# joedownard/skill-chaining-with-graphs

Measured on AMD Instinct MI355X. Metric: env-steps/sec (whole node), 65 536 parallel Pinball envs at 1/2/4/8 MI355X, higher is better.
Workload: dtype f32

## Files before the change

skill-chaining-with-graphs_amd/csrc/scg_kernels.hip:

```cpp
#include "scg_device.hpp"
#include "../../include/scg_abi.h"
#include <cstdio>
#include <cstdlib>
#include <cstring>
#include <cmath>
#include <mutex>
#include <new>
#include <type_traits>
#include <vector>

using namespace scg;
typedef float f4v __attribute__((ext_vector_type(4)));
typedef unsigned u4v __attribute__((ext_vector_type(4)));

#include "scg_eval.hpp"
#include "scg_step_kernel.hpp"
#include "scg_rollout_kernel.hpp"
#include "scg_trial_kernel.hpp"
#include "scg_order.hpp"
#include "scg_collect_kernels.hpp"
#include "scg_reduce_kernel.hpp"
#include "scg_apply_kernels.hpp"
#include "scg_aux_kernels.hpp"

// ... 142 lines not shown
    if (!c || !c->h_async) return 0;
    const uint32_t w = *reinterpret_cast<volatile uint32_t *>(c->h_async);
    if (w == 0) return 0;
    decode_async(w, c->err, sizeof(c->err));
    return 1;
}

extern "C" {

int scg_abi_version(void) { return SCG_ABI_VERSION; }

int scg_decode_async_word(uint32_t word, char *buf, int32_t buf_len) {
    return decode_async(word, buf, buf_len > 0 ? (size_t)buf_len : 0);
}

int scg_async_status(scg_ctx *c, void *stream, int32_t synchronize, uint32_t *word_out) {
    if (!c) return fail(nullptr, SCG_ERR_INVALID, "scg_async_status: null ctx");
    if (synchronize) {
        SCG_ON_DEVICE(c, "scg_async_status");
        SCG_HIP(c, hipStreamSynchronize(reinterpret_cast<hipStream_t>(stream)));
    }
    const uint32_t w = c->h_async ? *reinterpret_cast<volatile uint32_t *>(c->h_async) : 0u;
    if (word_out) *word_out = w;
    return decode_async(w, c->err, sizeof(c->err));
}

int scg_clear_async_error(scg_ctx *c) {
    if (!c) return fail(nullptr, SCG_ERR_INVALID, "scg_clear_async_error: null ctx");
    if (c->h_async) *reinterpret_cast<volatile uint32_t *>(c->h_async) = 0u;
    if (c->d_fail) {
        DeviceGuard g(c->cfg.device);
        if (g.ok) (void)hipMemset(c->d_fail, 0, sizeof(int32_t));
    }
    c->order_valid = false; c->hist_dirty = true; c->arm_rows_ready = false;
    return SCG_OK;
}

static int set_timeout(scg_ctx *c, const char *fn, double scg_ctx::*field, double seconds) {
    if (!c) return fail_in(nullptr, SCG_ERR_INVALID, fn, "null ctx");
    if (!(seconds >= 0.0) || seconds > 3600.0) return fail_in(c, SCG_ERR_INVALID, fn, "seconds must be in [0, 3600]");
    c->*field = seconds;
    return SCG_OK;
}

int scg_set_fit_timeout(scg_ctx *c, double seconds) { return set_timeout(c, "scg_set_fit_timeout", &scg_ctx::fit_timeout_s, seconds); }

int scg_set_peer_timeout(scg_ctx *c, double seconds) { return set_timeout(c, "scg_set_peer_timeout", &scg_ctx::peer_timeout_s, seconds); }

int scg_debug_raise_async(scg_ctx *c, uint32_t word) {
    if (!c || !c->h_async) return fail(c, SCG_ERR_INVALID, "scg_debug_raise_async: null ctx");
    *reinterpret_cast<volatile uint32_t *>(c->h_async) |= word;
    return SCG_OK;
}

int scg_block_envs(void) { return BLOCK_ENVS; }

const char *scg_strerror(int status) {
    switch (status) {
        case SCG_OK: return "ok";
        case SCG_ERR_INVALID: return "invalid argument";
        case SCG_ERR_NO_DEVICE: return "no usable HIP device";
        case SCG_ERR_HIP: return "HIP runtime error";
        case SCG_ERR_STATE: return "call order / state error";
        case SCG_ERR_ASYNC: return "an earlier launch failed on the device";
        default: return "unknown status";
    }
}

const char *scg_last_error(const scg_ctx *ctx) { return ctx ? ctx->err : g_err; }

static size_t hist_bytes(const scg_ctx *c) { return (size_t)((c->cfg.n_envs + 255) / 256) * HSTRIDE * sizeof(int32_t); }

struct CtxAlloc { void **ptr; size_t bytes; bool zero; };
static std::vector<CtxAlloc> ctx_allocs(scg_ctx *c) {
    auto P = [](auto **p) { return reinterpret_cast<void **>(p); };
    const size_t w = (size_t)c->n_vf * NACT * NF * sizeof(float), npos = (size_t)c->nblk * BLOCK_ENVS;
    const size_t rows = (size_t)(c->cfg.n_envs + COL_ROW - 1) / COL_ROW + 1;
    return {
        {P(&c->d_slabs), (size_t)c->nblk * w, false},
        {P(&c->d_cnts), (size_t)c->nblk * c->n_vf * sizeof(int32_t), true},
        {P(&c->d_G), w, true},
        {P(&c->d_nk), MAX_VF * sizeof(int32_t), true},
        {P(&c->d_edges), MAX_EDGES * 8 * sizeof(float), false},
        {P(&c->d_scale), NF * sizeof(float), false},
        {P(&c->d_perm), npos * sizeof(int32_t), false},
        {P(&c->d_hist), hist_bytes(c), false},
        {P(&c->d_collect_rows), rows * sizeof(int32_t), false},
        {P(&c->d_frontier_rows), MAX_VF * rows * sizeof(int32_t), false},
        {P(&c->d_fit_part), (size_t)FIT_BATCH * 2 * FIT_G * 8 * sizeof(unsigned long long), false},
        {P(&c->d_fail), sizeof(int32_t), true},
        {P(&c->d_outrec), npos * OREC * sizeof(float4), false},
        {P(&c->d_qalt), npos * 2 * sizeof(float4), false},
        {P(&c->d_invperm), npos * sizeof(int32_t), false},
        {P(&c->d_hist2[0]), hist_bytes(c), true},
        {P(&c->d_hist2[1]), hist_bytes(c), true},
        {P(&c->d_cellmask), (size_t)CELL_G * CELL_G * 4 * sizeof(uint64_t), false},
    };
}

#ifdef SCG_REDUCE_STAMPS
static size_t reduce_stamp_bytes(const scg_ctx *c) {
    const int nrow = (c->cfg.n_envs + 255) / 256, sy = (nrow + RED_NCOL - 1) / RED_NCOL;
    return (size_t)RED_NCOL * (c->n_vf + sy) * RED_STAMP_SLOTS * sizeof(unsigned long long);
}
#endif

int scg_create(scg_ctx **out, const scg_config *cfg) {
    if (!out || !cfg) return fail(nullptr, SCG_ERR_INVALID, "scg_create: null argument");
    *out = nullptr;
    if (cfg->n_envs < 1) return fail(nullptr, SCG_ERR_INVALID, "scg_create: n_envs must be >= 1");
    if (cfg->n_options < 0 || cfg->n_options > SCG_MAX_OPTIONS)
        return fail(nullptr, SCG_ERR_INVALID, "scg_create: n_options out of range [0,5]");
    if (cfg->update_count_floor < 0) return fail(nullptr, SCG_ERR_INVALID, "scg_create: update_count_floor must be >= 0");
    if (cfg->reoffer_period != 0 && !pow2(cfg->reoffer_period))
        return fail(nullptr, SCG_ERR_INVALID, "scg_create: reoffer_period must be a power of two (or 0)");
    if (cfg->fourier_order != SCG_FOURIER_ORDER)
        return fail(nullptr, SCG_ERR_INVALID, "scg_create: only Fourier order 5 is built");
    int ndev = 0;
    if (hipGetDeviceCount(&ndev) != hipSuccess || ndev < 1)
        return fail(nullptr, SCG_ERR_NO_DEVICE, "scg_create: no HIP device visible");
    if (cfg->device < 0 || cfg->device >= ndev)
        return fail(nullptr, SCG_ERR_INVALID, "scg_create: device ordinal out of range");
    scg_ctx *c = new (std::nothrow) scg_ctx();
    if (!c) return fail(nullptr, SCG_ERR_INVALID, "scg_create: out of host memory");
    memset(c, 0, sizeof(*c));
    c->cfg = *cfg;
    c->n_vf = cfg->n_options + 1;
    c->nblk = (cfg->n_envs + BLOCK_ENVS - 1) / BLOCK_ENVS;
    if (hipDeviceGetAttribute(&c->n_cu, hipDeviceAttributeMultiprocessorCount, cfg->device) != hipSuccess || c->n_cu <= 0) c->n_cu = 256;
    int st = SCG_OK;
    DeviceGuard dev_guard_(cfg->device);
    do {
        if (!dev_guard_.ok) { st = SCG_ERR_HIP; break; }
        for (const CtxAlloc &a : ctx_allocs(c)) {
            if (hipMalloc(a.ptr, a.bytes) != hipSuccess || (a.zero && hipMemset(*a.ptr, 0, a.bytes) != hipSuccess)) { st = SCG_ERR_HIP; break; }
        }
        if (st != SCG_OK) break;
        if (hipHostMalloc(reinterpret_cast<void **>(&c->h_async), 64, hipHostMallocMapped) != hipSuccess) { st = SCG_ERR_HIP; break; }
        *c->h_async = 0u;
        if (hipHostGetDevicePointer(reinterpret_cast<void **>(&c->d_async), c->h_async, 0) != hipSuccess) { st = SCG_ERR_HIP; break; }
    } while (0);
    if (st != SCG_OK) {
        snprintf(g_err, 256, "scg_create: device allocation/setup failed: %s", hipGetErrorString(hipGetLastError()));
        scg_destroy(c);
        return st;
    }
#ifdef SCG_STAMPS_LITE
    if (hipMalloc(&c->d_stamps, (size_t)c->nblk * STAMP_SLOTS * sizeof(unsigned long long)) == hipSuccess)
        (void)hipMemset(c->d_stamps, 0, (size_t)c->nblk * STAMP_SLOTS * sizeof(unsigned long long));
#endif
#ifdef SCG_REDUCE_STAMPS
    if (hipMalloc(&c->d_stamps, reduce_stamp_bytes(c)) == hipSuccess) (void)hipMemset(c->d_stamps, 0, reduce_stamp_bytes(c));
#endif
    c->parents = 0;
    for (int k = 1; k < MAX_VF; ++k) c->parents |= (uint32_t)(k - 1) << (3 * k);
    c->G_out = c->d_G; c->nk_out = c->d_nk;
    c->fit_timeout_s = 2.0;
    c->peer_timeout_s = 2.0;
    *out = c;
    return SCG_OK;
}

int scg_destroy(scg_ctx *c) {
    if (!c) return SCG_OK;
    for (const CtxAlloc &a : ctx_allocs(c)) (void)hipFree(*a.ptr);
    (void)hipFree(c->d_starts);
    if (c->h_async) (void)hipHostFree(c->h_async);
    if (c->peer_region) {
        DeviceGuard g(c->cfg.device);
        for (int r = 0; r < PEER_MAX; ++r)
            if (c->peer_mapped[r]) (void)hipIpcCloseMemHandle(c->peer_base[r]);
        {
            std::lock_guard<std::mutex> lk(g_peer_mu);
            for (size_t i = 0; i < g_peer_regions.size(); ++i)
                if (g_peer_regions[i].second == c->peer_region) { g_peer_regions.erase(g_peer_regions.begin() + i); break; }
        }
        (void)hipFree(c->peer_region); (void)hipFree(c->d_peer_go);
    }
    if (c->prof_ev) {
        for (hipEvent_t e : *c->prof_ev) (void)hipEventDestroy(e);
        delete c->prof_ev;
    }
    delete c;
    return SCG_OK;
}

int scg_set_hparams(scg_ctx *c, float gamma, float alpha, float epsilon, float r_option_success,
                    int32_t max_episode_steps, int32_t max_option_steps, int32_t update_count_floor, int32_t reoffer_period) {
    if (!c) return fail(nullptr, SCG_ERR_INVALID, "scg_set_hparams: null ctx");
    if (update_count_floor < 0) return fail(c, SCG_ERR_INVALID, "scg_set_hparams: update_count_floor must be >= 0");
    if (reoffer_period != 0 && !pow2(reoffer_period)) return fail(c, SCG_ERR_INVALID, "scg_set_hparams: reoffer_period must be a power of two (or 0)");
    c->cfg.gamma = gamma; c->cfg.alpha = alpha; c->cfg.epsilon = epsilon;
    c->cfg.r_option_success = r_option_success;
    c->cfg.max_episode_steps = max_episode_steps; c->cfg.max_option_steps = max_option_steps;
    c->cfg.update_count_floor = update_count_floor;
    c->cfg.reoffer_period = reoffer_period;
    return SCG_OK;
}

int scg_set_map(scg_ctx *c, const float *edges, int32_t n_edges, const float *starts, int32_t n_starts,
                const float map_scalars[6], const float *scale) {
    if (!c) return fail(nullptr, SCG_ERR_INVALID, "scg_set_map: null ctx");
    if (!edges || !starts || !map_scalars || !scale) return fail(c, SCG_ERR_INVALID, "scg_set_map: null argument");
    if (n_edges < 0 || n_edges > MAX_EDGES) return fail(c, SCG_ERR_INVALID, "scg_set_map: n_edges out of range [0,256]");
    if (n_starts < 1) return fail(c, SCG_ERR_INVALID, "scg_set_map: need at least one start position");
    SCG_ON_DEVICE(c, "scg_set_map");
    if (c->d_starts) { (void)hipFree(c->d_starts); c->d_starts = nullptr; }
    SCG_HIP(c, hipMalloc(&c->d_starts, (size_t)n_starts * 2 * sizeof(float)));
    if (n_edges > 0) SCG_HIP(c, hipMemcpy(c->d_edges, edges, (size_t)n_edges * 8 * sizeof(float), hipMemcpyHostToDevice));
    SCG_HIP(c, hipMemcpy(c->d_starts, starts, (size_t)n_starts * 2 * sizeof(float), hipMemcpyHostToDevice));
    SCG_HIP(c, hipMemcpy(c->d_scale, scale, NF * sizeof(float), hipMemcpyHostToDevice));
    const float R = map_scalars[0];
    c->ms.hstep = map_scalars[1]; c->ms.R2 = map_scalars[2];
    c->ms.TX = map_scalars[3]; c->ms.TY = map_scalars[4]; c->ms.TR2 = map_scalars[5];
    c->ms.R = R; c->ms.TR = (float)(std::sqrt((double)map_scalars[5]) * 1.0001);
    {
        std::vector<uint64_t> cm((size_t)CELL_G * CELL_G * 4, 0);
        const double vmax = 2.0 * std::sqrt(2.0) * 1.001;
        const double reach = (double)R * (1.02 + 1.10 * vmax) * 1.01 + 0.5 * std::sqrt(2.0) / CELL_G + 1e-6;
        for (int cy = 0; cy < CELL_G; ++cy)
            for (int cx = 0; cx < CELL_G; ++cx) {
                const double px = (cx + 0.5) / CELL_G, py = (cy + 0.5) / CELL_G;
                for (int j = 0; j < n_edges; ++j) {
                    const float *E = edges + 8 * j;
                    const double dx = px - E[0], dy = py - E[1];
                    double t = (dx * E[2] + dy * E[3]) * E[4];
                    t = t < 0 ? 0 : (t > 1 ? 1 : t);
                    const double qx = E[0] + E[2] * t - px, qy = E[1] + E[3] * t - py;
                    if (std::sqrt(qx * qx + qy * qy) <= reach)
                        cm[((size_t)cy * CELL_G + cx) * 4 + (j >> 6)] |= (1ull << (j & 63));
                }
            }
        SCG_HIP(c, hipMemcpy(c->d_cellmask, cm.data(), cm.size() * sizeof(uint64_t), hipMemcpyHostToDevice));
    }
    c->ms.n_edges = n_edges; c->ms.n_starts = n_starts;
    c->have_map = true;
    return SCG_OK;
}

struct PeerTarget {
    scg_ctx *c;
    float *G, *nkf;
    int32_t *nk;
    explicit PeerTarget(scg_ctx *ctx) : c(ctx), G(ctx->G_out), nkf(ctx->nkf_out), nk(ctx->nk_out) {
        if (!c->peer_n) return;
        float *op = reinterpret_cast<float *>(c->peer_region + PEER_HDR + (c->peer_e & 1u) * c->peer_op_stride);
        c->G_out = op; c->nkf_out = op + (size_t)c->n_vf * NACT * NF; c->nk_out = c->d_nk;
    }
    ~PeerTarget() { c->G_out = G; c->nkf_out = nkf; c->nk_out = nk; }
};

extern "C++" template <typename Args>
static void fill_shared(const scg_ctx *c, Args &A) {
    memset(&A, 0, sizeof(A));
    A.n = c->cfg.n_envs; A.n_vf = c->n_vf;
    A.seed = c->cfg.seed; A.env_base = c->cfg.env_id_base;
    A.epsilon = c->cfg.epsilon; A.max_ep = c->cfg.max_episode_steps; A.max_opt = c->cfg.max_option_steps;
    A.reoffer_mask = c->cfg.reoffer_period > 1 ? (uint32_t)(c->cfg.reoffer_period - 1) : 0u;
    A.parents = c->parents; A.gest = c->gest;
    A.ms = c->ms;
    A.edges = c->d_edges; A.starts = c->d_starts; A.cellmask = c->d_cellmask;
}

static void fill_common(const scg_ctx *c, StepArgs &A) {
    fill_shared(c, A);
    A.gamma = c->cfg.gamma; A.r_succ = c->cfg.r_option_success;
    A.slabs = c->d_slabs; A.cnts = c->d_cnts;
    A.gest_succ = c->gest_succ;
    A.ring_x = c->ring_x; A.ring_y = c->ring_y; A.events = c->events; A.ev_len = c->ev_len;
    A.ring_mask = c->ring_len > 0 ? c->ring_len - 1 : 0;
    A.stamps = c->d_stamps;
    A.async_word = c->d_async; A.fail_flag = c->d_fail;
}

enum ReduceMode { REDUCE_ONLY, COMMIT_ONLY, REDUCE_COMMIT, REDUCE_COMMIT_SORT };
static int launch_reduce(scg_ctx *c, float *W, uint32_t apply, int nblk, hipStream_t s, ReduceMode mode, const StepArgs *st = nullptr) {
    ReduceArgs R;
    memset(&R, 0, sizeof(R));
    R.slabs = c->d_slabs; R.cnts = c->d_cnts; R.G = c->G_out; R.n_k = c->nk_out; R.nk_f = c->nkf_out; R.W = W; R.scale = c->d_scale;
    R.nblk = nblk; R.n_vf = c->n_vf; R.alpha = c->cfg.alpha; R.apply = apply; R.fail_flag = c->d_fail; R.nk_floor = c->cfg.update_count_floor;
    const int nrow = st ? (c->cfg.n_envs + 255) / 256 : 0;
    R.n = c->cfg.n_envs; R.nrow = nrow;
    if (st) {
        R.outrec = c->d_outrec; R.qalt = c->d_qalt; R.invperm = c->d_invperm; R.perm = c->d_perm; R.sort = mode == REDUCE_COMMIT_SORT ? 1 : 0;
        R.hist = c->d_hist2[c->hist_parity]; R.hist_zero = c->d_hist2[c->hist_parity ^ 1];
        R.x = st->x; R.y = st->y; R.vx = st->vx; R.vy = st->vy; R.reward = st->reward;
        R.option_id_out = st->option_id; R.opt_steps = st->opt_steps; R.ep_steps = st->ep_steps;
        R.action = st->action; R.done = st->done;
        R.qcache = st->k_hi >= 0 ? st->qcache : nullptr;
        if (c->arm_bits && c->events && c->ring_x) {
            R.c_events = c->events; R.c_prev = c->arm_prev; R.c_evlen = c->ev_len; R.c_count = c->arm_count;
            R.c_rows = c->d_collect_rows; R.c_bits = c->arm_bits; R.c_L = c->arm_L; R.c_ring_len = c->ring_len;
        }
    }
#ifdef SCG_REDUCE_STAMPS
    R.stamps = c->d_stamps;
#endif
    if (mode == COMMIT_ONLY) {
        hipLaunchKernelGGL(commit_kernel, dim3(nrow), dim3(256), 0, s, R);
        SCG_HIP(c, hipGetLastError());
        return SCG_OK;
    }
    const int sy = (nrow + RED_NCOL - 1) / RED_NCOL;
    if (RED_NCOL * (c->n_vf + sy) <= c->n_cu)
        hipLaunchKernelGGL(reduce_kernel<16>, dim3(RED_NCOL, c->n_vf + sy), dim3(RED_THREADS), 0, s, R);
    else
        hipLaunchKernelGGL(reduce_kernel<8>, dim3(RED_NCOL, c->n_vf + sy), dim3(RED_THREADS), 0, s, R);
    SCG_HIP(c, hipGetLastError());
    return SCG_OK;
}

static int sort_env_order(scg_ctx *c, const int32_t *option_id, hipStream_t s) {
    if (c->order_valid && c->order_ids == option_id) return SCG_OK;
    const int nrow = (c->cfg.n_envs + 255) / 256;
    hipLaunchKernelGGL(sort_hist_kernel, dim3(nrow), dim3(256), 0, s, option_id, c->cfg.n_envs, c->n_vf, c->d_hist);
    hipLaunchKernelGGL(sort_scatter_kernel, dim3(nrow), dim3(256), 0, s, option_id, c->cfg.n_envs, c->n_vf, nrow,
                       c->d_hist, c->d_perm, c->d_invperm);
    SCG_HIP(c, hipGetLastError());
    return SCG_OK;
}

static int prof_begin(scg_ctx *c, hipStream_t s, hipEvent_t &ev1) {
    if (!(c->prof_on && (c->prof_seen++ % c->prof_every) == c->prof_every / 2)) return SCG_OK;
    if (!c->prof_ev) c->prof_ev = new std::vector<hipEvent_t>();
    while (c->prof_ev->size() < c->prof_used + 2) {
        hipEvent_t e;
        SCG_HIP(c, hipEventCreate(&e));
        c->prof_ev->push_back(e);
    }
    hipEvent_t ev0 = (*c->prof_ev)[c->prof_used];
    ev1 = (*c->prof_ev)[c->prof_used + 1];
    c->prof_used += 2;
    SCG_HIP(c, hipEventRecord(ev0, s));
    return SCG_OK;
}

int scg_step(scg_ctx *c, float *x, float *y, float *vx, float *vy, int32_t *option_id, int32_t *opt_steps,
             int32_t *ep_steps, float *qcache, uint8_t *action, float *reward, uint8_t *done, float *W,
             const float *clf, uint32_t enabled_mask, uint64_t t, uint32_t flags, void *stream) {
    if (!c) return fail(nullptr, SCG_ERR_INVALID, "scg_step: null ctx");
    if (!c->have_map) return fail(c, SCG_ERR_STATE, "scg_step: scg_set_map has not been called");
    if (!x || !y || !vx || !vy || !option_id || !opt_steps || !ep_steps || !qcache || !action || !reward ||
        !done || !W || !clf)
        return fail(c, SCG_ERR_INVALID, "scg_step: null array argument");
    if (c->peer_n && (flags & SCG_STEP_LEARN) && (flags & SCG_STEP_APPLY))
        return fail(c, SCG_ERR_INVALID, "scg_step: SCG_STEP_APPLY with a peer region open (the update is scg_peer_exchange_apply's)");
    if ((flags & SCG_STEP_INTERRUPT) && !(flags & SCG_STEP_LEARN))
        return fail(c, SCG_ERR_INVALID, "scg_step: SCG_STEP_INTERRUPT without SCG_STEP_LEARN (acting-only interruption is scg_rollout_interrupt)");
    SCG_CHECK_ASYNC(c);
    SCG_ON_DEVICE(c, "scg_step");
    if (c->arm_bits) {
        const void *ptrs[2] = {c->arm_count, c->arm_prev};
        for (const void *p : ptrs) {
            if (!p) continue;
            hipPointerAttribute_t at;
            if (hipPointerGetAttributes(&at, p) != hipSuccess || at.type != hipMemoryTypeDevice) {
                (void)hipGetLastError();
                c->arm_bits = 0; c->arm_rows_ready = false;
                return fail(c, SCG_ERR_STATE, "scg_step: the buffers announced with scg_arm_collect are no longer device memory "
                                              "(freed before scg_arm_collect(0)?); the trigger has been disarmed");
            }
        }
    }
    hipStream_t s = reinterpret_cast<hipStream_t>(stream);
    StepArgs A;
    fill_common(c, A);
    A.x = x; A.y = y; A.vx = vx; A.vy = vy;
    A.option_id = option_id; A.opt_steps = opt_steps; A.ep_steps = ep_steps; A.qcache = qcache;
    A.action = action; A.reward = reward; A.done = done;
    A.W = W; A.clf = clf;
    A.k_lo = 0; A.k_hi = c->n_vf - 1;
    A.enabled = enabled_mask; A.learn = (flags & SCG_STEP_LEARN) ? 1u : 0u; A.t = t;
    if (flags & 0x100u) A.k_hi = -1;
    if (const int rc = sort_env_order(c, option_id, s)) return rc;
    c->order_valid = false;
    if (c->hist_dirty) {
        const size_t hb = hist_bytes(c);
        SCG_HIP(c, hipMemsetAsync(c->d_hist2[0], 0, hb, s));
        SCG_HIP(c, hipMemsetAsync(c->d_hist2[1], 0, hb, s));
        c->hist_dirty = false;
    }
    const bool fold = (flags & SCG_STEP_LEARN) && !(flags & 0x200u);
    A.hist_next = fold ? c->d_hist2[c->hist_parity] : nullptr;
    A.perm = c->d_perm; A.outrec = c->d_outrec; A.qalt = c->d_qalt;
    hipEvent_t ev1 = nullptr;
    if (const int rc = prof_begin(c, s, ev1)) return rc;
    if (flags & SCG_STEP_INTERRUPT)
        hipLaunchKernelGGL(td_kernel<MODE_FUSED_INT>, dim3(c->nblk), dim3(THREADS), 0, s, A);
    else
        hipLaunchKernelGGL(td_kernel<MODE_FUSED>, dim3(c->nblk), dim3(THREADS), 0, s, A);
    SCG_HIP(c, hipGetLastError());
    if (ev1) SCG_HIP(c, hipEventRecord(ev1, s));
    c->arm_rows_ready = c->arm_bits && c->events && c->ring_x;
    if (!(flags & SCG_STEP_LEARN)) return launch_reduce(c, W, 0u, c->nblk, s, COMMIT_ONLY, &A);
    PeerTarget peer_target(c);
    if (!fold) return launch_reduce(c, W, (flags & SCG_STEP_APPLY) ? 1u : 0u, c->nblk, s, REDUCE_COMMIT, &A);
    c->hist_dirty = true;
    const int rc = launch_reduce(c, W, (flags & SCG_STEP_APPLY) ? 1u : 0u, c->nblk, s, REDUCE_COMMIT_SORT, &A);
    if (rc != SCG_OK) return rc;
    c->hist_dirty = false;
    c->hist_parity ^= 1;
    c->order_valid = true; c->order_ids = option_id;
    return SCG_OK;
}

static bool rollout_epw(const scg_ctx *c, int n, int &epw) {
    epw = 2;
    while (epw < RO_MAX_EPW && (long long)n >= (long long)c->n_cu * RO_WAVES * epw * 2) epw *= 2;
    if (const char *ov = getenv("SCG_ROLLOUT_EPW")) {
        const int v = atoi(ov);
        if (v < 2 || v > RO_MAX_EPW || !pow2(v)) return false;
        epw = v;
    }
    return true;
}

static int check_record(scg_ctx *c, const char *fn, const scg_record *rec, int N, long long min_rows) {
    const char *why = !rec->len ? "rec->len is required" : rec->n < 1 ? "rec->n must be >= 1"
                    : rec->first < 0 || (long long)rec->first + rec->n > N ? "rec->first .. first+n-1 outside the envs / entries"
                    : rec->rows < min_rows ? "rec->rows too small for the launch's pseudo-steps" : nullptr;
    return why ? fail_in(c, SCG_ERR_INVALID, fn, why) : SCG_OK;
}

extern "C++" template <typename Derived, typename Base, typename Set>
static Derived derived_args(const Base &base, Set set) {
    Derived D;
    memset(&D, 0, sizeof(D));
    static_cast<Base &>(D) = base;
    set(D);
    return D;
}

static int rollout_launch(const char *fn, scg_ctx *c, float *x, float *y, float *vx, float *vy, int32_t *option_id, int32_t *opt_steps,
                          int32_t *ep_steps, float *qcache, uint8_t *action, float *reward, uint8_t *done,
                          const float *W, const float *clf, uint32_t enabled_mask, uint64_t t0, int32_t n_steps,
                          uint32_t flags, const scg_rollout_stats *stats, const scg_record *rec, bool at, void *stream,
                          bool intr = false, int32_t *interrupts = nullptr, bool best = false, int32_t *overrides = nullptr) {
    if (!c) return fail_in(nullptr, SCG_ERR_INVALID, fn, "null ctx");
    if (!c->have_map) return fail_in(c, SCG_ERR_STATE, fn, "scg_set_map has not been called");
    if (!x || !y || !vx || !vy || !option_id || !opt_steps || !ep_steps || !qcache || !action || !reward ||
        !done || !W || !clf)
        return fail_in(c, SCG_ERR_INVALID, fn, "null array argument");
    if (flags & ~(SCG_ROLLOUT_BEGIN | SCG_ROLLOUT_ONE_EPISODE)) return fail_in(c, SCG_ERR_INVALID, fn, "unknown flag");
    if (n_steps < 0 || n_steps > SCG_ROLLOUT_MAX_STEPS)
        return fail_in(c, SCG_ERR_INVALID, fn, "n_steps out of range [0, SCG_ROLLOUT_MAX_STEPS]");
    if (n_steps == 0 && !(flags & SCG_ROLLOUT_BEGIN))
        return fail_in(c, SCG_ERR_INVALID, fn, "n_steps == 0 without SCG_ROLLOUT_BEGIN (or _BEGIN_AT)");
    if ((flags & SCG_ROLLOUT_ONE_EPISODE) && !(stats && stats->finished))
        return fail_in(c, SCG_ERR_INVALID, fn, "SCG_ROLLOUT_ONE_EPISODE needs stats->finished");
    if (rec) {
        const int rc = check_record(c, fn, rec, c->cfg.n_envs, (long long)n_steps + ((flags & SCG_ROLLOUT_BEGIN) ? 1 : 0));
        if (rc != SCG_OK) return rc;
    }
    SCG_CHECK_ASYNC(c);
    DeviceGuard dev_guard_(c->cfg.device);
    if (!dev_guard_.ok) return fail_in(c, SCG_ERR_HIP, fn, "cannot make the context's device current");
    RolloutArgs R;
    fill_shared(c, R);
    R.x = x; R.y = y; R.vx = vx; R.vy = vy; R.option_id = option_id; R.opt_steps = opt_steps; R.ep_steps = ep_steps;
    R.qcache = qcache; R.action = action; R.reward = reward; R.done = done; R.W = W; R.clf = clf;
    if (stats) R.st = *stats;
    R.n_steps = n_steps;
    R.begin = (flags & SCG_ROLLOUT_BEGIN) ? 1u : 0u; R.one_episode = (flags & SCG_ROLLOUT_ONE_EPISODE) ? 1u : 0u;
    R.enabled = enabled_mask; R.t0 = t0;
    int epw;
    if (!rollout_epw(c, c->cfg.n_envs, epw)) return fail_in(c, SCG_ERR_INVALID, fn, "SCG_ROLLOUT_EPW must be 2, 4, 8, 16 or 32");
    R.epw = epw;
    const int grid = (c->cfg.n_envs + RO_WAVES * epw - 1) / (RO_WAVES * epw);
    c->order_valid = false;
    if (best) {
        const auto fill = [&](auto &D) { if (rec) D.rec = *rec; D.begin_at = at ? 1u : 0u; D.interrupts = interrupts; D.overrides = overrides; };
        if (intr) SCG_HIP(c, launch_rollout_best_interrupt(derived_args<RolloutBestIntArgs>(R, fill), grid, reinterpret_cast<hipStream_t>(stream)));
        else SCG_HIP(c, launch_rollout_best(derived_args<RolloutBestArgs>(R, fill), grid, reinterpret_cast<hipStream_t>(stream)));
    } else if (intr && (rec || at)) {
        const auto RR = derived_args<RolloutIntRecArgs>(R, [&](auto &D) { if (rec) D.rec = *rec; D.begin_at = at ? 1u : 0u; D.interrupts = interrupts; });
        SCG_HIP(c, launch_rollout_interrupt_record(RR, grid, reinterpret_cast<hipStream_t>(stream)));
    } else if (intr) {
        const auto RI = derived_args<RolloutIntArgs>(R, [&](auto &D) { D.interrupts = interrupts; });
        SCG_HIP(c, launch_rollout_interrupt(RI, grid, reinterpret_cast<hipStream_t>(stream)));
    } else if (rec || at) {
        const auto RR = derived_args<RolloutRecArgs>(R, [&](auto &D) { if (rec) D.rec = *rec; D.begin_at = at ? 1u : 0u; });
        SCG_HIP(c, launch_rollout_record(RR, grid, reinterpret_cast<hipStream_t>(stream)));
    } else {
        hipLaunchKernelGGL((rollout_kernel<false, RolloutArgs>), dim3(grid), dim3(RO_THREADS), 0, reinterpret_cast<hipStream_t>(stream), R);
        SCG_HIP(c, hipGetLastError());
    }
    return SCG_OK;
}

int scg_rollout(scg_ctx *c, float *x, float *y, float *vx, float *vy, int32_t *option_id, int32_t *opt_steps,
                int32_t *ep_steps, float *qcache, uint8_t *action, float *reward, uint8_t *done,
                const float *W, const float *clf, uint32_t enabled_mask, uint64_t t0, int32_t n_steps,
                uint32_t flags, const scg_rollout_stats *stats, void *stream) {
    return rollout_launch("scg_rollout", c, x, y, vx, vy, option_id, opt_steps, ep_steps, qcache, action, reward, done, W, clf,
                          enabled_mask, t0, n_steps, flags, stats, nullptr, false, stream);
}

static int begin_at_flags(scg_ctx *c, const char *fn, uint32_t &flags, bool &at) {
    at = (flags & SCG_ROLLOUT_BEGIN_AT) != 0;
    if (c && at && (flags & SCG_ROLLOUT_BEGIN))
        return fail_in(c, SCG_ERR_INVALID, fn, "SCG_ROLLOUT_BEGIN and SCG_ROLLOUT_BEGIN_AT together");
    if (at) flags = (flags & ~SCG_ROLLOUT_BEGIN_AT) | SCG_ROLLOUT_BEGIN;
    return SCG_OK;
}

int scg_rollout_record(scg_ctx *c, float *x, float *y, float *vx, float *vy, int32_t *option_id, int32_t *opt_steps,
                       int32_t *ep_steps, float *qcache, uint8_t *action, float *reward, uint8_t *done,
                       const float *W, const float *clf, uint32_t enabled_mask, uint64_t t0, int32_t n_steps,
                       uint32_t flags, const scg_rollout_stats *stats, const scg_record *rec, void *stream) {
    bool at;
    if (const int rc = begin_at_flags(c, "scg_rollout_record", flags, at)) return rc;
    return rollout_launch("scg_rollout_record", c, x, y, vx, vy, option_id, opt_steps, ep_steps, qcache, action, reward, done,
                          W, clf, enabled_mask, t0, n_steps, flags, stats, rec, at, stream);
}

int scg_rollout_interrupt(scg_ctx *c, float *x, float *y, float *vx, float *vy, int32_t *option_id, int32_t *opt_steps,
                          int32_t *ep_steps, float *qcache, uint8_t *action, float *reward, uint8_t *done,
                          const float *W, const float *clf, uint32_t enabled_mask, uint64_t t0, int32_t n_steps,
                          uint32_t flags, const scg_rollout_stats *stats, int32_t *interrupts, const scg_record *rec,
                          void *stream) {
    bool at;
    if (const int rc = begin_at_flags(c, "scg_rollout_interrupt", flags, at)) return rc;
    return rollout_launch("scg_rollout_interrupt", c, x, y, vx, vy, option_id, opt_steps, ep_steps, qcache, action, reward, done,
                          W, clf, enabled_mask, t0, n_steps, flags, stats, rec, at, stream, true, interrupts);
}

int scg_rollout_select(scg_ctx *c, float *x, float *y, float *vx, float *vy, int32_t *option_id, int32_t *opt_steps,
                       int32_t *ep_steps, float *qcache, uint8_t *action, float *reward, uint8_t *done,
                       const float *W, const float *clf, uint32_t enabled_mask, uint64_t t0, int32_t n_steps,
                       uint32_t flags, const scg_rollout_stats *stats, int32_t *interrupts, int32_t *overrides,
                       const scg_record *rec, uint32_t rules, void *stream) {
    if (c && (rules & ~(SCG_SELECT_INTERRUPT | SCG_SELECT_BEST)))
        return fail_in(c, SCG_ERR_INVALID, "scg_rollout_select", "unknown rule");
    const bool intr = (rules & SCG_SELECT_INTERRUPT) != 0, best = (rules & SCG_SELECT_BEST) != 0;
    bool at;
    if (const int rc = begin_at_flags(c, "scg_rollout_select", flags, at)) return rc;
    return rollout_launch("scg_rollout_select", c, x, y, vx, vy, option_id, opt_steps, ep_steps, qcache, action, reward, done,
                          W, clf, enabled_mask, t0, n_steps, flags, stats, rec, at, stream, intr, intr ? interrupts : nullptr,
                          best, best ? overrides : nullptr);
}

static int trials_launch(const char *fn, scg_ctx *c, int32_t n, const float *x, const float *y, const float *vx, const float *vy,
                         const int32_t *option, const float *W, const float *clf, uint32_t enabled_mask, uint64_t t0,
                         const scg_trial_out *out, const scg_record *rec, void *stream) {
    if (!c) return fail_in(nullptr, SCG_ERR_INVALID, fn, "null ctx");
    if (!c->have_map) return fail_in(c, SCG_ERR_STATE, fn, "scg_set_map has not been called");
    if (!x || !y || !vx || !vy || !option || !W || !clf || !out || !out->outcome)
        return fail_in(c, SCG_ERR_INVALID, fn, "null array argument (or out->outcome)");
    if (n < 1) return fail_in(c, SCG_ERR_INVALID, fn, "n must be >= 1");
    if (std::min(c->cfg.max_option_steps, c->cfg.max_episode_steps) > SCG_TRIAL_MAX_STEPS)
        return fail_in(c, SCG_ERR_INVALID, fn, "min(max_option_steps, max_episode_steps) exceeds SCG_TRIAL_MAX_STEPS");
    if (rec) {
        const int rc = check_record(c, fn, rec, n, 1);
        if (rc != SCG_OK) return rc;
    }
    SCG_CHECK_ASYNC(c);
    DeviceGuard dev_guard_(c->cfg.device);
    if (!dev_guard_.ok) return fail_in(c, SCG_ERR_HIP, fn, "cannot make the context's device current");
    TrialArgs T;
    fill_shared(c, T);
    T.n = n;
    T.x = x; T.y = y; T.vx = vx; T.vy = vy; T.option = option; T.out = *out; T.W = W; T.clf = clf;
    T.enabled = enabled_mask; T.t0 = t0;
    T.gamma = c->cfg.gamma; T.r_succ = c->cfg.r_option_success;
    int epw;
    if (!rollout_epw(c, n, epw)) return fail_in(c, SCG_ERR_INVALID, fn, "SCG_ROLLOUT_EPW must be 2, 4, 8, 16 or 32");
    T.epw = epw;
    const int grid = (int)(((long long)n + RO_WAVES * epw - 1) / (RO_WAVES * epw));
    if (rec) {
        const auto TR = derived_args<TrialRecArgs>(T, [&](auto &D) { D.rec = *rec; });
        SCG_HIP(c, launch_trial_record(TR, grid, reinterpret_cast<hipStream_t>(stream)));
    } else {
        hipLaunchKernelGGL((trial_kernel<false, TrialArgs>), dim3(grid), dim3(RO_THREADS), 0, reinterpret_cast<hipStream_t>(stream), T);
        SCG_HIP(c, hipGetLastError());
    }
    return SCG_OK;
}

int scg_option_trials(scg_ctx *c, int32_t n, const float *x, const float *y, const float *vx, const float *vy,
                      const int32_t *option, const float *W, const float *clf, uint32_t enabled_mask, uint64_t t0,
                      const scg_trial_out *out, void *stream) {
    return trials_launch("scg_option_trials", c, n, x, y, vx, vy, option, W, clf, enabled_mask, t0, out, nullptr, stream);
}

int scg_option_trials_record(scg_ctx *c, int32_t n, const float *x, const float *y, const float *vx, const float *vy,
                             const int32_t *option, const float *W, const float *clf, uint32_t enabled_mask, uint64_t t0,
                             const scg_trial_out *out, const scg_record *rec, void *stream) {
    return trials_launch("scg_option_trials_record", c, n, x, y, vx, vy, option, W, clf, enabled_mask, t0, out, rec, stream);
}

int scg_invalidate_order(scg_ctx *c) {
    if (!c) return fail(nullptr, SCG_ERR_INVALID, "scg_invalidate_order: null ctx");
    c->order_valid = false;
    return SCG_OK;
}

#ifdef SCG_STAMPS_LITE
extern "C" int scg_diag_stamps(scg_ctx *c, unsigned long long *host_out , int32_t reset) {
    if (!c || !c->d_stamps) return SCG_ERR_STATE;
    if (host_out && hipMemcpy(host_out, c->d_stamps, (size_t)c->nblk * STAMP_SLOTS * sizeof(unsigned long long), hipMemcpyDeviceToHost) != hipSuccess) return SCG_ERR_HIP;
    if (reset) (void)hipMemset(c->d_stamps, 0, (size_t)c->nblk * STAMP_SLOTS * sizeof(unsigned long long));
    return SCG_OK;
}
#endif

#ifdef SCG_REDUCE_STAMPS
extern "C" int scg_diag_reduce_stamps(scg_ctx *c, unsigned long long *host_out, int32_t reset) {
// ... 421 lines not shown
```

skill-chaining-with-graphs_amd/csrc/scg_reduce_kernel.hpp:

```cpp
#pragma once

struct ReduceArgs {
    const float *slabs;
    const int32_t *cnts;
    float *G;
    int32_t *n_k;
    float *nk_f;
    float *W;
    const float *scale;
    int32_t nblk, n_vf;
    float alpha;
    uint32_t apply;
    int32_t nk_floor;
    const int32_t *option_id;
    int32_t *hist, *hist_zero, *perm;
    int32_t n, nrow;
    const float4 *outrec;
    const float4 *qalt;
    int32_t *invperm;
    float *x, *y, *vx, *vy, *reward;
    int32_t *option_id_out, *opt_steps, *ep_steps;
    uint8_t *action, *done;
    float *qcache;
    int32_t sort;
    const int32_t *fail_flag;
    const uint8_t *c_events, *c_prev;
    const int32_t *c_evlen, *c_count;
    int32_t *c_rows;
    uint32_t c_bits;
    int32_t c_L, c_ring_len;
#ifdef SCG_REDUCE_STAMPS
    unsigned long long *stamps;
#endif
};

constexpr int SEG = 16;
constexpr int RED_WAVES = 16;
constexpr int RED_THREADS = 64 * RED_WAVES;
constexpr int RED_SPW = 2;
constexpr int RED_COLS = NACT * NF / 4;
constexpr int RED_NCOL = (RED_COLS + 63) / 64;
constexpr int RED_STAMP_SLOTS = 8;

__device__ __forceinline__ void commit_and_place_row(const ReduceArgs &R, int row, int wv, int lane, int (*s_x)[40]) {
    int zoff = 0;
    asm volatile("" : "+v"(zoff));
    const int step_failed = R.fail_flag[zoff];
    const bool act = wv < 4 && row < R.nrow;
    const int e = row * 256 + wv * 64 + lane;
    const bool ok = act && e < R.n;
    const int pos_old = ok ? R.invperm[e] : 0;
    int tot[NKEY], pre[NKEY];
#pragma unroll
    for (int k = 0; k < NKEY; ++k) { tot[k] = 0; pre[k] = 0; }
    if (act && R.sort) {
        for (int r = wv * 64 + lane; r < R.nrow; r += 256) {
#pragma unroll
            for (int k = 0; k < NKEY; ++k) {
                const int h = R.hist[r * HSTRIDE + k];
                tot[k] += h;
                if (r < row) pre[k] += h;
            }
        }
    }
    float4 ra = make_float4(0.0f, 0.0f, 0.0f, 0.0f), rb = ra, rq = ra;
    float q4 = 0.0f;
    if (ok) {
        const float4 *r = R.outrec + (size_t)pos_old * OREC;
        const float4 r3 = r[3];
        ra = r[0]; rb = r[1]; rq = r[2]; q4 = r3.x;
        if (__float_as_uint(r3.y) == OREC_DECLINED) {
            rq = R.qalt[(size_t)pos_old * 2]; q4 = R.qalt[(size_t)pos_old * 2 + 1].x;
            rb.y = __uint_as_float(__float_as_uint(rb.y) | 0x01000000u);
        }
    }
    int key = -1;
    uint64_t km[NKEY];
    if (act) {
        if (R.sort) {
#pragma unroll
            for (int k = 0; k < NKEY; ++k) {
#pragma unroll
                for (int m = 1; m < 64; m <<= 1) { tot[k] += __shfl_xor(tot[k], m, 64); pre[k] += __shfl_xor(pre[k], m, 64); }
            }
        }
        const unsigned bits = __float_as_uint(rb.y);
        if (ok && !step_failed) {
            const int on = (int)((bits >> 16) & 255u);
            const bool declined = (bits >> 24) & 1u;
            const int oid = declined ? -on : (on ? on : -(int)((bits >> 28) & 7u));
            key = sort_key(oid, R.n_vf);
            R.x[e] = ra.x; R.y[e] = ra.y; R.vx[e] = ra.z; R.vy[e] = ra.w;
            R.reward[e] = rb.x; R.action[e] = (uint8_t)(bits & 255u); R.done[e] = (uint8_t)((bits >> 8) & 255u);
            R.option_id_out[e] = oid; R.opt_steps[e] = __float_as_int(rb.z); R.ep_steps[e] = __float_as_int(rb.w);
            if (R.qcache) {
                const size_t n = (size_t)R.n;
                R.qcache[e] = rq.x; R.qcache[n + e] = rq.y; R.qcache[2 * n + e] = rq.z;
                R.qcache[3 * n + e] = rq.w; R.qcache[4 * n + e] = q4;
            }
        }
        if (R.sort) {
#pragma unroll
            for (int k = 0; k < NKEY; ++k) km[k] = __ballot(key == k);
            if (lane < 3 * NKEY) {
                int v = 0;
#pragma unroll
                for (int k = 0; k < NKEY; ++k) {
                    if (lane == k) v = tot[k];
                    if (lane == NKEY + k) v = pre[k];
                    if (lane == 2 * NKEY + k) v = __popcll(km[k]);
                }
                s_x[wv][lane] = v;
            }
        }
    }
    if (R.c_rows && act) {
        bool in;
        int v = collect_v(e, R.n, R.c_events, R.c_prev, R.c_bits, R.c_evlen, R.c_ring_len, R.c_L, in);
#pragma unroll
        for (int m = 1; m < 64; m <<= 1) v += __shfl_xor(v, m, 64);
        if (lane == 0) s_x[wv][3 * NKEY] = v;
    }
    if (!R.sort && !R.c_rows) return;
    __syncthreads();
    if (R.c_rows && wv == 0 && lane == 0 && row < R.nrow) {
        R.c_rows[row] = s_x[0][3 * NKEY] + s_x[1][3 * NKEY] + s_x[2][3 * NKEY] + s_x[3][3 * NKEY];
        if (row == 0) R.c_rows[R.nrow] = *R.c_count;
    }
    if (!R.sort || !act) return;
    int off[NKEY];
#pragma unroll
    for (int k = 0; k < NKEY; ++k) {
        tot[k] = s_x[0][k] + s_x[1][k] + s_x[2][k] + s_x[3][k];
        off[k] = s_x[0][NKEY + k] + s_x[1][NKEY + k] + s_x[2][NKEY + k] + s_x[3][NKEY + k];
#pragma unroll
        for (int w = 0; w < 3; ++w) off[k] += w < wv ? s_x[w][2 * NKEY + k] : 0;
    }
    OrderLayout L;
    order_layout(tot, R.n, L);
    int rk = -1, st = 0;
#pragma unroll
    for (int k = 0; k < NKEY; ++k)
        if (key == k) { rk = off[k] + __popcll(km[k] & ((1ull << lane) - 1ull)); st = L.start[k]; }
    if (rk >= 0 && !step_failed) {
        const int pos = key == 0 ? order_pos0(L, rk) : order_posk(L, st, rk);
        R.perm[pos] = e; R.invperm[e] = pos;
    }
    if (wv == 0 && lane < HSTRIDE) R.hist_zero[row * HSTRIDE + lane] = 0;
}

__device__ __forceinline__ int lane_now() {
    int ln;
    asm volatile("v_mbcnt_lo_u32_b32 %0, -1, 0\n\tv_mbcnt_hi_u32_b32 %0, -1, %0" : "=v"(ln));
    return ln;
}

__device__ __forceinline__ int row_sum(int v) {
    v += __builtin_amdgcn_mov_dpp(v, 0xB1, 0xF, 0xF, true);
    v += __builtin_amdgcn_mov_dpp(v, 0x4E, 0xF, 0xF, true);
    v += __builtin_amdgcn_mov_dpp(v, 0x141, 0xF, 0xF, true);
    v += __builtin_amdgcn_mov_dpp(v, 0x140, 0xF, 0xF, true);
    return v;
}

#ifdef SCG_REDUCE_STAMPS
#define RED_STAMP(slot) do { \
        if (R.stamps && lane_now() == 0) \
            R.stamps[(size_t)__builtin_amdgcn_readfirstlane((int)(blockIdx.y * gridDim.x + blockIdx.x) * RED_STAMP_SLOTS + (slot))] = __builtin_amdgcn_s_memrealtime(); \
    } while (0)
#define RED_STAMP_DRAINED(slot) do { asm volatile("s_waitcnt vmcnt(0) lgkmcnt(0)" ::: "memory"); RED_STAMP(slot); } while (0)
#else
#define RED_STAMP(slot) do { } while (0)
#define RED_STAMP_DRAINED(slot) do { } while (0)
#endif

template <int BATCH>
__global__ __launch_bounds__(RED_THREADS, BATCH == 16 ? 4 : 8) void reduce_kernel(const ReduceArgs R) {
    __shared__ float4 s_T[RED_WAVES * RED_SPW][64];
    __shared__ int s_cnt[RED_WAVES * RED_SPW];
    __shared__ int s_x[4][40];
    const int sy_rows = (int)gridDim.y - R.n_vf;
    const int wave = __builtin_amdgcn_readfirstlane((int)threadIdx.x >> 6);
    RED_STAMP(0);
    if ((int)blockIdx.y < sy_rows) {
        const int row = (int)blockIdx.y * (int)gridDim.x + blockIdx.x;
        commit_and_place_row(R, row, wave, threadIdx.x & 63, s_x);
        if (wave < 4) RED_STAMP_DRAINED(1 + wave);
        return;
    }
    const int k = (int)blockIdx.y - sy_rows;
    const size_t slab_stride = (size_t)R.n_vf * RED_COLS * sizeof(float4);
    const char *slab_k = reinterpret_cast<const char *>(R.slabs) + (size_t)k * RED_COLS * sizeof(float4);
    const int nseg = (R.nblk + SEG - 1) / SEG;
    float4 S = make_float4(0.0f, 0.0f, 0.0f, 0.0f);
    int nk = 0;
    float4 w_old = make_float4(0.0f, 0.0f, 0.0f, 0.0f), sc = w_old;
    int step_failed = 0;
    for (int sg0 = 0; sg0 < nseg; sg0 += RED_WAVES * RED_SPW) {
        const int lane = lane_now();
        int cs[RED_SPW];
#pragma unroll
        for (int j = 0; j < RED_SPW; ++j) {
            const int bl = (sg0 + j * RED_WAVES + wave) * SEG + (lane & (SEG - 1));
            cs[j] = R.cnts[(unsigned)(min(bl, R.nblk - 1) * R.n_vf + k)];
        }
#pragma unroll
        for (int j = 0; j < RED_SPW; ++j) {
            const int b0 = (sg0 + j * RED_WAVES + wave) * SEG;
            const int c = (lane < SEG && b0 + lane < R.nblk) ? cs[j] : 0;
            const unsigned mask = (unsigned)__ballot(c > 0);
            float4 T = make_float4(0.0f, 0.0f, 0.0f, 0.0f);
            if (mask) {
                const __amdgpu_buffer_rsrc_t seg = __builtin_amdgcn_make_buffer_rsrc(
                    const_cast<char *>(slab_k + (size_t)b0 * slab_stride), 0, 0x7fffffff, 0x00020000);
                const int i4 = blockIdx.x * 64 + lane;
                const unsigned col_off = (unsigned)(i4 < RED_COLS ? i4 : 0) * (unsigned)sizeof(float4);
#pragma unroll
                for (int h = 0; h < SEG; h += BATCH) {
                    if (!((mask >> h) & ((1u << BATCH) - 1u))) continue;
                    u4v v[BATCH];
#pragma unroll
                    for (int u = 0; u < BATCH; ++u) {
                        v[u] = (u4v){0u, 0u, 0u, 0u};
                        if ((mask >> (h + u)) & 1u) v[u] = __builtin_amdgcn_raw_buffer_load_b128(seg, (int)col_off, (int)((h + u) * (unsigned)slab_stride), 0);
                    }
#pragma unroll
                    for (int u = 0; u < BATCH; ++u) {
                        if ((mask >> (h + u)) & 1u) {
                            T.x = T.x + __uint_as_float(v[u][0]); T.y = T.y + __uint_as_float(v[u][1]);
                            T.z = T.z + __uint_as_float(v[u][2]); T.w = T.w + __uint_as_float(v[u][3]);
                        }
                    }
                }
            }
            __builtin_amdgcn_s_waitcnt(0x0F70);
            s_T[j * RED_WAVES + wave][lane] = T;
            const int ctot = row_sum(c);
            if (lane == 0) s_cnt[j * RED_WAVES + wave] = ctot;
        }
        const bool last = sg0 + RED_WAVES * RED_SPW >= nseg;
        if (wave == 0 && last) RED_STAMP(5);
        if (wave == 0 && R.apply && last) {
            step_failed = *R.fail_flag;
            const int i4 = blockIdx.x * 64 + lane_now();
            const int col = i4 < RED_COLS ? i4 : 0;
            w_old = reinterpret_cast<const float4 *>(R.W)[(size_t)k * RED_COLS + col];
            sc = *reinterpret_cast<const float4 *>(R.scale + (col * 4) % NF);
        }
        __syncthreads();
        if (wave == 0) {
            if (last) RED_STAMP(6);
            const int ln = lane_now();
            const int cu = row_sum(ln < RED_WAVES * RED_SPW ? s_cnt[ln] : 0);
            nk += __builtin_amdgcn_readlane(cu, 0) + __builtin_amdgcn_readlane(cu, 16);
#pragma unroll
            for (int h = 0; h < RED_WAVES * RED_SPW; h += BATCH) {
                float4 t[BATCH];
#pragma unroll
                for (int u = 0; u < BATCH; ++u) t[u] = s_T[h + u][ln];
#pragma unroll
                for (int u = 0; u < BATCH; ++u) { S.x = S.x + t[u].x; S.y = S.y + t[u].y; S.z = S.z + t[u].z; S.w = S.w + t[u].w; }
            }
            if (last) RED_STAMP(7);
        }
        if (!last) __syncthreads();
    }
    if (wave != 0) return;
    const int lane = lane_now(), i4 = blockIdx.x * 64 + lane;
    if (blockIdx.x == 0 && lane == 0) {
        R.n_k[k] = nk;
        if (R.nk_f) R.nk_f[k] = (float)nk;
    }
    if (i4 >= RED_COLS) return;
    reinterpret_cast<float4 *>(R.G)[(size_t)k * RED_COLS + i4] = S;
    if (R.apply && nk > 0 && !step_failed) {
        const float step = R.alpha / (float)max(nk, R.nk_floor);
        float4 w = w_old;
        w.x = fmaf(step * sc.x, S.x, w.x); w.y = fmaf(step * sc.y, S.y, w.y);
        w.z = fmaf(step * sc.z, S.z, w.z); w.w = fmaf(step * sc.w, S.w, w.w);
        reinterpret_cast<float4 *>(R.W)[(size_t)k * RED_COLS + i4] = w;
    }
    RED_STAMP_DRAINED(1);
}

__global__ __launch_bounds__(256) void commit_kernel(const ReduceArgs R) {
    __shared__ int s_x[4][40];
    commit_and_place_row(R, blockIdx.x, threadIdx.x >> 6, threadIdx.x & 63, s_x);
}
```

Baseline: 885.2 million.

## Narrow reduce column tiles to 16 lanes and use DPP/permlane sums in commit

```diff
diff --git a/skill-chaining-with-graphs_amd/csrc/scg_kernels.hip b/skill-chaining-with-graphs_amd/csrc/scg_kernels.hip
--- a/skill-chaining-with-graphs_amd/csrc/scg_kernels.hip
+++ b/skill-chaining-with-graphs_amd/csrc/scg_kernels.hip
@@ -468,7 +468,8 @@
         return SCG_OK;
     }
     const int sy = (nrow + RED_NCOL - 1) / RED_NCOL;
-    if (RED_NCOL * (c->n_vf + sy) <= c->n_cu)
+    constexpr int W64 = (RED_COLS + 63) / 64;
+    if (W64 * (c->n_vf + (nrow + W64 - 1) / W64) <= c->n_cu)
         hipLaunchKernelGGL(reduce_kernel<16>, dim3(RED_NCOL, c->n_vf + sy), dim3(RED_THREADS), 0, s, R);
     else
         hipLaunchKernelGGL(reduce_kernel<8>, dim3(RED_NCOL, c->n_vf + sy), dim3(RED_THREADS), 0, s, R);
diff --git a/skill-chaining-with-graphs_amd/csrc/scg_reduce_kernel.hpp b/skill-chaining-with-graphs_amd/csrc/scg_reduce_kernel.hpp
--- a/skill-chaining-with-graphs_amd/csrc/scg_reduce_kernel.hpp
+++ b/skill-chaining-with-graphs_amd/csrc/scg_reduce_kernel.hpp
@@ -35,12 +35,48 @@
 };
 
 constexpr int SEG = 16;
-constexpr int RED_WAVES = 16;
+constexpr int RED_ROUND = 32;
+constexpr int RED_SPW = 2;
+constexpr int RED_GROUPS = RED_ROUND / RED_SPW;
+constexpr int RED_COLS = NACT * NF / 4;
+constexpr int RED_C = 16;
+constexpr int RED_GPW = 64 / RED_C;
+constexpr int RED_WAVES = RED_GROUPS / RED_GPW;
 constexpr int RED_THREADS = 64 * RED_WAVES;
-constexpr int RED_SPW = 2;
-constexpr int RED_COLS = NACT * NF / 4;
-constexpr int RED_NCOL = (RED_COLS + 63) / 64;
-constexpr int RED_STAMP_SLOTS = 8;
+constexpr int RED_NCOL = (RED_COLS + RED_C - 1) / RED_C;
+constexpr int RED_STAMP_SLOTS = 24;
+
+__device__ __forceinline__ int lane_now() {
+    int ln;
+    asm volatile("v_mbcnt_lo_u32_b32 %0, -1, 0\n\tv_mbcnt_hi_u32_b32 %0, -1, %0" : "=v"(ln));
+    return ln;
+}
+
+__device__ __forceinline__ int row_sum(int v) {
+    v += __builtin_amdgcn_mov_dpp(v, 0xB1, 0xF, 0xF, true);
+    v += __builtin_amdgcn_mov_dpp(v, 0x4E, 0xF, 0xF, true);
+    v += __builtin_amdgcn_mov_dpp(v, 0x141, 0xF, 0xF, true);
+    v += __builtin_amdgcn_mov_dpp(v, 0x140, 0xF, 0xF, true);
+    return v;
+}
+
+__device__ __forceinline__ int rows_sum(int v) {
+    const auto h = __builtin_amdgcn_permlane32_swap((unsigned)v, (unsigned)v, false, false);
+    v = (int)(h[0] + h[1]);
+    const auto q = __builtin_amdgcn_permlane16_swap((unsigned)v, (unsigned)v, false, false);
+    return (int)(q[0] + q[1]);
+}
+
+#ifdef SCG_REDUCE_STAMPS
+#define RED_STAMP(slot) do { \
+        if (R.stamps && lane_now() == 0) \
+            R.stamps[(size_t)__builtin_amdgcn_readfirstlane((int)(blockIdx.y * gridDim.x + blockIdx.x) * RED_STAMP_SLOTS + (slot))] = __builtin_amdgcn_s_memrealtime(); \
+    } while (0)
+#define RED_STAMP_DRAINED(slot) do { asm volatile("s_waitcnt vmcnt(0) lgkmcnt(0)" ::: "memory"); RED_STAMP(slot); } while (0)
+#else
+#define RED_STAMP(slot) do { } while (0)
+#define RED_STAMP_DRAINED(slot) do { } while (0)
+#endif
 
 __device__ __forceinline__ void commit_and_place_row(const ReduceArgs &R, int row, int wv, int lane, int (*s_x)[40]) {
     int zoff = 0;
@@ -49,7 +85,7 @@
     const bool act = wv < 4 && row < R.nrow;
     const int e = row * 256 + wv * 64 + lane;
     const bool ok = act && e < R.n;
-    const int pos_old = ok ? R.invperm[e] : 0;
+    const unsigned pos_old = (unsigned)*(ok ? R.invperm + e : R.fail_flag);
     int tot[NKEY], pre[NKEY];
 #pragma unroll
     for (int k = 0; k < NKEY; ++k) { tot[k] = 0; pre[k] = 0; }
@@ -63,27 +99,38 @@
             }
         }
     }
-    float4 ra = make_float4(0.0f, 0.0f, 0.0f, 0.0f), rb = ra, rq = ra;
-    float q4 = 0.0f;
+    float4 ra = make_float4(0.0f, 0.0f, 0.0f, 0.0f), rb = ra, rq = ra, r3 = ra, qa = ra;
+    float qb = 0.0f;
     if (ok) {
         const float4 *r = R.outrec + (size_t)pos_old * OREC;
-        const float4 r3 = r[3];
-        ra = r[0]; rb = r[1]; rq = r[2]; q4 = r3.x;
-        if (__float_as_uint(r3.y) == OREC_DECLINED) {
-            rq = R.qalt[(size_t)pos_old * 2]; q4 = R.qalt[(size_t)pos_old * 2 + 1].x;
-            rb.y = __uint_as_float(__float_as_uint(rb.y) | 0x01000000u);
-        }
+        const float4 *q = R.qalt + (size_t)pos_old * 2;
+        ra = r[0]; rb = r[1]; rq = r[2]; r3 = r[3];
+        qa = q[0]; qb = q[1].x;
+    }
+    int tsum = 0;
+    if (act && R.sort) {
+        const int j = lane & 15;
+#pragma unroll
+        for (int k = 0; k < NKEY; ++k) {
+            const int t = row_sum(tot[k]), p = row_sum(pre[k]);
+            if (j == k) tsum = t;
+            if (j == NKEY + k) tsum = p;
+        }
+        tsum = rows_sum(tsum);
+    }
+#ifdef SCG_REDUCE_STAMPS
+    if (wv == 0 && act) { asm volatile("s_waitcnt vmcnt(0)" ::: "memory"); RED_STAMP(5); }
+#endif
+    unsigned mark = __float_as_uint(r3.y);
+    asm volatile("" : "+v"(mark), "+v"(tsum) : "v"(r3.z), "v"(r3.w), "v"(pos_old));
+    float q4 = r3.x;
+    if (ok && mark == OREC_DECLINED) {
+        rq = qa; q4 = qb;
+        rb.y = __uint_as_float(__float_as_uint(rb.y) | 0x01000000u);
     }
     int key = -1;
     uint64_t km[NKEY];
     if (act) {
-        if (R.sort) {
-#pragma unroll
-            for (int k = 0; k < NKEY; ++k) {
-#pragma unroll
-                for (int m = 1; m < 64; m <<= 1) { tot[k] += __shfl_xor(tot[k], m, 64); pre[k] += __shfl_xor(pre[k], m, 64); }
-            }
-        }
         const unsigned bits = __float_as_uint(rb.y);
         if (ok && !step_failed) {
             const int on = (int)((bits >> 16) & 255u);
@@ -103,26 +150,24 @@
 #pragma unroll
             for (int k = 0; k < NKEY; ++k) km[k] = __ballot(key == k);
             if (lane < 3 * NKEY) {
-                int v = 0;
-#pragma unroll
-                for (int k = 0; k < NKEY; ++k) {
-                    if (lane == k) v = tot[k];
-                    if (lane == NKEY + k) v = pre[k];
+                int v = tsum;
+#pragma unroll
+                for (int k = 0; k < NKEY; ++k)
                     if (lane == 2 * NKEY + k) v = __popcll(km[k]);
-                }
                 s_x[wv][lane] = v;
             }
         }
     }
     if (R.c_rows && act) {
         bool in;
-        int v = collect_v(e, R.n, R.c_events, R.c_prev, R.c_bits, R.c_evlen, R.c_ring_len, R.c_L, in);
-#pragma unroll
-        for (int m = 1; m < 64; m <<= 1) v += __shfl_xor(v, m, 64);
+        const int v = rows_sum(row_sum(collect_v(e, R.n, R.c_events, R.c_prev, R.c_bits, R.c_evlen, R.c_ring_len, R.c_L, in)));
         if (lane == 0) s_x[wv][3 * NKEY] = v;
     }
     if (!R.sort && !R.c_rows) return;
-    __syncthreads();
+    asm volatile("s_waitcnt lgkmcnt(0)\n\ts_barrier" ::: "memory");
+#ifdef SCG_REDUCE_STAMPS
+    if (wv == 0 && act) RED_STAMP(6);
+#endif
     if (R.c_rows && wv == 0 && lane == 0 && row < R.nrow) {
         R.c_rows[row] = s_x[0][3 * NKEY] + s_x[1][3 * NKEY] + s_x[2][3 * NKEY] + s_x[3][3 * NKEY];
         if (row == 0) R.c_rows[R.nrow] = *R.c_count;
@@ -149,35 +194,11 @@
     if (wv == 0 && lane < HSTRIDE) R.hist_zero[row * HSTRIDE + lane] = 0;
 }
 
-__device__ __forceinline__ int lane_now() {
-    int ln;
-    asm volatile("v_mbcnt_lo_u32_b32 %0, -1, 0\n\tv_mbcnt_hi_u32_b32 %0, -1, %0" : "=v"(ln));
-    return ln;
-}
-
-__device__ __forceinline__ int row_sum(int v) {
-    v += __builtin_amdgcn_mov_dpp(v, 0xB1, 0xF, 0xF, true);
-    v += __builtin_amdgcn_mov_dpp(v, 0x4E, 0xF, 0xF, true);
-    v += __builtin_amdgcn_mov_dpp(v, 0x141, 0xF, 0xF, true);
-    v += __builtin_amdgcn_mov_dpp(v, 0x140, 0xF, 0xF, true);
-    return v;
-}
-
-#ifdef SCG_REDUCE_STAMPS
-#define RED_STAMP(slot) do { \
-        if (R.stamps && lane_now() == 0) \
-            R.stamps[(size_t)__builtin_amdgcn_readfirstlane((int)(blockIdx.y * gridDim.x + blockIdx.x) * RED_STAMP_SLOTS + (slot))] = __builtin_amdgcn_s_memrealtime(); \
-    } while (0)
-#define RED_STAMP_DRAINED(slot) do { asm volatile("s_waitcnt vmcnt(0) lgkmcnt(0)" ::: "memory"); RED_STAMP(slot); } while (0)
-#else
-#define RED_STAMP(slot) do { } while (0)
-#define RED_STAMP_DRAINED(slot) do { } while (0)
-#endif
-
 template <int BATCH>
 __global__ __launch_bounds__(RED_THREADS, BATCH == 16 ? 4 : 8) void reduce_kernel(const ReduceArgs R) {
-    __shared__ float4 s_T[RED_WAVES * RED_SPW][64];
-    __shared__ int s_cnt[RED_WAVES * RED_SPW];
+    constexpr int C = RED_C, GPW = RED_GPW;
+    __shared__ float4 s_T[RED_ROUND][C];
+    __shared__ int s_cnt[RED_ROUND];
     __shared__ int s_x[4][40];
     const int sy_rows = (int)gridDim.y - R.n_vf;
     const int wave = __builtin_amdgcn_readfirstlane((int)threadIdx.x >> 6);
@@ -196,37 +217,44 @@
     int nk = 0;
     float4 w_old = make_float4(0.0f, 0.0f, 0.0f, 0.0f), sc = w_old;
     int step_failed = 0;
-    for (int sg0 = 0; sg0 < nseg; sg0 += RED_WAVES * RED_SPW) {
+    for (int sg0 = 0; sg0 < nseg; sg0 += RED_ROUND) {
         const int lane = lane_now();
+        const int grp = wave * GPW + lane / C;
         int cs[RED_SPW];
 #pragma unroll
         for (int j = 0; j < RED_SPW; ++j) {
-            const int bl = (sg0 + j * RED_WAVES + wave) * SEG + (lane & (SEG - 1));
+            const int bl = (sg0 + j * RED_GROUPS + grp) * SEG + (lane & (SEG - 1));
             cs[j] = R.cnts[(unsigned)(min(bl, R.nblk - 1) * R.n_vf + k)];
         }
 #pragma unroll
         for (int j = 0; j < RED_SPW; ++j) {
-            const int b0 = (sg0 + j * RED_WAVES + wave) * SEG;
-            const int c = (lane < SEG && b0 + lane < R.nblk) ? cs[j] : 0;
-            const unsigned mask = (unsigned)__ballot(c > 0);
+            const int b0w = (sg0 + j * RED_GROUPS + wave * GPW) * SEG;
+            const int c = ((sg0 + j * RED_GROUPS + grp) * SEG + (lane & (SEG - 1)) < R.nblk) ? cs[j] : 0;
+            const uint64_t ball = __ballot(c > 0);
+            unsigned mask, any;
+            static_assert(C == 16, "a lane group is a row of 16 lanes: its blocks are its row's bits of the ballot");
+            mask = (unsigned)(ball >> (lane & 48)) & 0xffffu;
+            any = (unsigned)(ball | (ball >> 16) | (ball >> 32) | (ball >> 48)) & 0xffffu;
             float4 T = make_float4(0.0f, 0.0f, 0.0f, 0.0f);
-            if (mask) {
+            if (any) {
                 const __amdgpu_buffer_rsrc_t seg = __builtin_amdgcn_make_buffer_rsrc(
-                    const_cast<char *>(slab_k + (size_t)b0 * slab_stride), 0, 0x7fffffff, 0x00020000);
-                const int i4 = blockIdx.x * 64 + lane;
-                const unsigned col_off = (unsigned)(i4 < RED_COLS ? i4 : 0) * (unsigned)sizeof(float4);
+                    const_cast<char *>(slab_k + (size_t)b0w * slab_stride), 0, 0x7fffffff, 0x00020000);
+                const int i4 = blockIdx.x * C + (lane & (C - 1));
+                unsigned col_off = (unsigned)(i4 < RED_COLS ? i4 : 0) * (unsigned)sizeof(float4);
+                col_off += (unsigned)(lane / C) * (unsigned)(SEG * slab_stride);
 #pragma unroll
                 for (int h = 0; h < SEG; h += BATCH) {
-                    if (!((mask >> h) & ((1u << BATCH) - 1u))) continue;
+                    if (!((any >> h) & ((1u << BATCH) - 1u))) continue;
                     u4v v[BATCH];
 #pragma unroll
                     for (int u = 0; u < BATCH; ++u) {
                         v[u] = (u4v){0u, 0u, 0u, 0u};
+                        if (!((any >> (h + u)) & 1u)) continue;
                         if ((mask >> (h + u)) & 1u) v[u] = __builtin_amdgcn_raw_buffer_load_b128(seg, (int)col_off, (int)((h + u) * (unsigned)slab_stride), 0);
                     }
 #pragma unroll
                     for (int u = 0; u < BATCH; ++u) {
-                        if ((mask >> (h + u)) & 1u) {
+                        if ((any >> (h + u)) & 1u) {
                             T.x = T.x + __uint_as_float(v[u][0]); T.y = T.y + __uint_as_float(v[u][1]);
                             T.z = T.z + __uint_as_float(v[u][2]); T.w = T.w + __uint_as_float(v[u][3]);
                         }
@@ -234,15 +262,17 @@
                 }
             }
             __builtin_amdgcn_s_waitcnt(0x0F70);
-            s_T[j * RED_WAVES + wave][lane] = T;
+            s_T[j * RED_GROUPS + grp][lane & (C - 1)] = T;
             const int ctot = row_sum(c);
-            if (lane == 0) s_cnt[j * RED_WAVES + wave] = ctot;
-        }
-        const bool last = sg0 + RED_WAVES * RED_SPW >= nseg;
+            if ((lane & (C - 1)) == 0) s_cnt[j * RED_GROUPS + grp] = ctot;
+        }
+        const bool last = sg0 + RED_ROUND >= nseg;
+        if (last) RED_STAMP(8 + wave);
         if (wave == 0 && last) RED_STAMP(5);
         if (wave == 0 && R.apply && last) {
             step_failed = *R.fail_flag;
-            const int i4 = blockIdx.x * 64 + lane_now();
+            const int ln = lane_now();
+            const int i4 = blockIdx.x * C + (ln & (C - 1));
             const int col = i4 < RED_COLS ? i4 : 0;
             w_old = reinterpret_cast<const float4 *>(R.W)[(size_t)k * RED_COLS + col];
             sc = *reinterpret_cast<const float4 *>(R.scale + (col * 4) % NF);
@@ -251,13 +281,14 @@
         if (wave == 0) {
             if (last) RED_STAMP(6);
             const int ln = lane_now();
-            const int cu = row_sum(ln < RED_WAVES * RED_SPW ? s_cnt[ln] : 0);
+            const int cl = ln & (C - 1);
+            const int cu = row_sum(ln < RED_ROUND ? s_cnt[ln] : 0);
             nk += __builtin_amdgcn_readlane(cu, 0) + __builtin_amdgcn_readlane(cu, 16);
 #pragma unroll
-            for (int h = 0; h < RED_WAVES * RED_SPW; h += BATCH) {
+            for (int h = 0; h < RED_ROUND; h += BATCH) {
                 float4 t[BATCH];
 #pragma unroll
-                for (int u = 0; u < BATCH; ++u) t[u] = s_T[h + u][ln];
+                for (int u = 0; u < BATCH; ++u) t[u] = s_T[h + u][cl];
 #pragma unroll
                 for (int u = 0; u < BATCH; ++u) { S.x = S.x + t[u].x; S.y = S.y + t[u].y; S.z = S.z + t[u].z; S.w = S.w + t[u].w; }
             }
@@ -266,12 +297,12 @@
         if (!last) __syncthreads();
     }
     if (wave != 0) return;
-    const int lane = lane_now(), i4 = blockIdx.x * 64 + lane;
+    const int lane = lane_now(), i4 = blockIdx.x * C + lane;
     if (blockIdx.x == 0 && lane == 0) {
         R.n_k[k] = nk;
         if (R.nk_f) R.nk_f[k] = (float)nk;
     }
-    if (i4 >= RED_COLS) return;
+    if (lane >= C || i4 >= RED_COLS) return;
     reinterpret_cast<float4 *>(R.G)[(size_t)k * RED_COLS + i4] = S;
     if (R.apply && nk > 0 && !step_failed) {
         const float step = R.alpha / (float)max(nk, R.nk_floor);
```

Measured after the change: 897.8 million (median of 6 runs). 1.4% higher.
